# mburger-stsci/nexoclom

Hardware: AMD Instinct MI355X
Metric: particle*steps/s (higher is better)
Workload: dtype f64

## Files before the change

### nexoclom_amd/csrc/nxc_api.hip

```cpp
#include <hip/hip_runtime.h>
#include <dlfcn.h>
#include <rccl/rccl.h>

#include <algorithm>
#include <atomic>
#include <cmath>
#include <cstddef>
#include <cstdio>
#include <cstdlib>
#include <cstring>
#include <ctime>
#include <limits>
#include <mutex>
#include <new>
#include <string>
#include <utility>
#include <vector>

#include "../../include/nexoclom_hip.h"
#include "nxc_camera_check.hpp"
#include "nxc_shell_check.hpp"
#include "nxc_cube_check.hpp"
#include "nxc_los_profile_check.hpp"
#include "nxc_desc_check.hpp"
// ... 2571 lines not shown
        K.n_node_az = rows(ST_NODE_AZ);
    }
    HIPCHK(hipMemsetAsync(h->d_ctr, 0, sizeof(DevCounters), h->stream));
    if ((rc = begin_timed(h))) return rc;
    const auto kernel = plan.law == NXC_LAW_NODES ? k_sample<NXC_LAW_NODES>
                        : (plan.law == NXC_LAW_THERMAL ? k_sample<NXC_LAW_THERMAL> : k_sample<NXC_LAW_PLAIN>);
    hipLaunchKernelGGL(kernel, dim3(flat_grid(h, n, NXC_BLOCK)), dim3(NXC_BLOCK), 0, h->stream, K, n,
                       h->d_packets, h->d_ctr);
    HIPCHK(hipGetLastError());
    if ((rc = end_timed(h))) return rc;
    DevCounters c;
    HIPCHK(hipMemcpyAsync(&c, h->d_ctr, sizeof c, hipMemcpyDeviceToHost, h->stream));
    HIPCHK(stream_sync(h));
    if (c.unfinished) {
        h->n_packets = 0;
        h->have_order = false;
        return fail(NXC_ERR_ARG, "nxc_packets_sample: " + std::to_string(c.unfinished) +
                                 " packets found no launch point in the density map (is it "
                                 "almost everywhere zero?)");
    }
    h->n_packets = total;
    h->var_n = -1;
    h->rows_total = -1;
    if (offset == 0) h->first_id = d->first_index;
    h->have_order = false;
    if (soa_out)
        HIPCHK(hipMemcpy2DAsync(soa_out, (size_t)n * 8, h->d_packets + offset, (size_t)total * 8,
                                (size_t)n * 8, 8, hipMemcpyDeviceToHost, h->stream));
    if (offset + n < total) {
        HIPCHK(stream_sync(h));
        return NXC_OK;
    }
    if ((rc = order_on_device(h, plan.k2max, nullptr, 0))) return rc;
    HIPCHK(stream_sync(h));
    return NXC_OK;
    });
}

int nxc_integrate_const_async(nxc_handle *h, double step, int64_t n_iter, double outeredge,
                              uint32_t flags)
{
    return guarded([&]() -> int {
    int rc = need_forces(h);
    if (rc) return rc;
    if (h->n_packets < 1) return fail(NXC_ERR_STATE, "no resident packets (nxc_packets_upload)");
    if (!(step > 0) || n_iter < 0) return fail(NXC_ERR_ARG, "step must be > 0, n_iter >= 0");
    const bool image = (flags & NXC_RUN_IMAGE) != 0;
    if (image && !h->have_image) return fail(NXC_ERR_STATE, "NXC_RUN_IMAGE without nxc_set_image");
    if ((rc = speed_order_for_const(h))) return rc;
    return launch_const(h, step, n_iter, outeredge, image, nullptr, nullptr);
    });
}

int nxc_integrate_const_streamed(nxc_handle *h, int64_t n, const double *soa0, int32_t pieces,
                                 double step, int64_t n_iter, double outeredge, uint32_t flags)
{
    return guarded([&]() -> int {
    int rc = need_forces(h);
    if (rc) return rc;
    if (n < 1 || !soa0 || pieces < 1 || pieces > 32) return fail(NXC_ERR_ARG, "bad arguments (1..32 pieces)");
    if (!(step > 0) || n_iter < 0) return fail(NXC_ERR_ARG, "step must be > 0, n_iter >= 0");
    const bool image = (flags & NXC_RUN_IMAGE) != 0;
    if (image && !h->have_image) return fail(NXC_ERR_STATE, "NXC_RUN_IMAGE without nxc_set_image");
    if (n >= (int64_t)0xffffffffll) return fail(NXC_ERR_ARG, "too many packets for one resident set");
    if (h->have_bodies || h->have_bounce)
        return fail(NXC_ERR_STATE, "the streamed pass covers the plain force models; with moons or "
                                   "surface re-emission upload first (nxc_packets_upload)");
    if ((int64_t)pieces > n) pieces = (int32_t)n;
    const size_t per_piece = NXC_ORDER_BINS + 8;
    if ((rc = h->d_packets.ensure((size_t)8 * n * 8))) return rc;
    if ((rc = h->d_queue.ensure((size_t)8 * n * 8))) return rc;
    if ((rc = h->d_order.ensure((size_t)n * sizeof(unsigned)))) return rc;
    if ((rc = h->d_piece_hist.ensure((32 * per_piece + 8) * sizeof(unsigned long long)))) return rc;
    for (int e = 0; e <= 32; e++)
        if (!h->ev_piece[e]) HIPCHK(hipEventCreateWithFlags(&h->ev_piece[e], hipEventDisableTiming));
    unsigned long long *d_avail = h->d_piece_hist + 32 * per_piece;
    h->n_packets = n;
    h->var_n = -1;
    h->first_id = 0;
    h->rows_total = -1;
    h->have_order = false;

    if ((rc = upload_step(h, step))) return rc;
    HIPCHK(hipMemsetAsync(h->d_ctr, 0, sizeof(DevCounters), h->stream));
    HIPCHK(hipMemsetAsync(d_avail, 0, sizeof(unsigned long long), h->stream));
    HIPCHK(hipEventRecord(h->ev_piece[32], h->stream));
    HIPCHK(hipStreamWaitEvent(h->stream2, h->ev_piece[32], 0));
    HIPCHK(hipStreamWaitEvent(h->copy_stream, h->ev_piece[32], 0));
    FusedJob job;
    job.soa = h->d_queue; job.order = h->d_order; job.avail = d_avail;
    if ((rc = launch_fused(h, image, 0, n_iter, outeredge, job))) return rc;
    auto give_up = [&](int code) {
        hipLaunchKernelGGL(k_publish, dim3(1), dim3(64), 0, h->stream2, d_avail, ~0ull);
        (void)hipStreamSynchronize(h->stream2);
        (void)stream_sync(h);
        h->n_packets = 0;
        return code;
    };
    std::vector<int64_t> bound((size_t)pieces + 1, n);
    bound[0] = 0;
    if (pieces > 1) {
        int64_t first = std::max<int64_t>(n / (4 * (int64_t)pieces), (int64_t)h->n_cu * BLOCK_PERSIST * 2);
        first = std::min(first, n / pieces);
        for (int p = 1; p < pieces; p++) bound[(size_t)p] = first + (n - first) * (p - 1) / (pieces - 1);
    }
    const bool withhold = std::getenv("NXC_TEST_WITHHOLD_LAST_PIECE") != nullptr;
    for (int p = 0; p < pieces; p++) {
        const int64_t p0 = bound[(size_t)p], len = bound[(size_t)p + 1] - p0;
        if (len <= 0) continue;
        if (withhold && p == pieces - 1 && pieces > 1) break;
        hipError_t e = hipSuccess;
        for (int c = 0; c < 8 && e == hipSuccess; c++)
            e = hipMemcpyAsync(h->d_packets + c * n + p0, soa0 + c * n + p0, (size_t)len * 8,
                               hipMemcpyHostToDevice, h->copy_stream);
        if (e == hipSuccess) e = hipEventRecord(h->ev_piece[p], h->copy_stream);
        if (e == hipSuccess) e = hipStreamWaitEvent(h->stream2, h->ev_piece[p], 0);
        unsigned long long *hist = h->d_piece_hist + (size_t)p * per_piece, *d_max = hist + NXC_ORDER_BINS;
        if (e == hipSuccess) e = hipMemsetAsync(d_max, 0, sizeof(unsigned long long), h->stream2);
        if (e != hipSuccess)
            return give_up(fail_hip("streamed upload", e));
        hipLaunchKernelGGL(k_speed_max<false>, dim3(flat_grid(h, len, NXC_BLOCK)), dim3(NXC_BLOCK), 0,
                           h->stream2, (const double *)(h->d_packets + p0), n, len, d_max);
        if ((rc = order_async(h, h->stream2, h->d_packets + p0, n, len, nullptr, 0.0, d_max, hist,
                              h->d_order + p0, h->d_queue + 8 * p0, true, (unsigned)p0)))
            return give_up(rc);
        hipLaunchKernelGGL(k_publish, dim3(1), dim3(64), 0, h->stream2, d_avail,
                           (unsigned long long)(p0 + len));
        if (hipGetLastError() != hipSuccess) return give_up(fail(NXC_ERR_HIP, "streamed upload: launch failed"));
    }
    h->have_order = true;
    h->order_key = 0;
    h->streamed_pending = true;
    HIPCHK(hipEventRecord(h->ev_piece[32], h->stream2));
    HIPCHK(hipStreamWaitEvent(h->stream, h->ev_piece[32], 0));
    return NXC_OK;
    });
}

int nxc_integrate_const(nxc_handle *h, double step, int64_t n_iter, double outeredge,
                        uint32_t flags, double *traj_out, int64_t nrec, double *final_out,
                        int64_t *steps_out)
{
    return guarded([&]() -> int {
    int rc = need_forces(h);
    if (rc) return rc;
    const int64_t n = h->n_packets;
    if (n < 1) return fail(NXC_ERR_STATE, "no resident packets (nxc_packets_upload)");
    if (!(step > 0) || n_iter < 0) return fail(NXC_ERR_ARG, "step must be > 0, n_iter >= 0");
    const bool image = (flags & NXC_RUN_IMAGE) != 0;
    if (image && !h->have_image) return fail(NXC_ERR_STATE, "NXC_RUN_IMAGE without nxc_set_image");
    if (traj_out && nrec < n_iter + 1) return fail(NXC_ERR_ARG, "nrec must be >= n_iter + 1");
    if ((rc = speed_order_for_const(h))) return rc;

    const size_t col = (size_t)n * sizeof(double);
    double *d_final = nullptr;
    long long *d_steps = nullptr;
    if (!traj_out) {
        if (final_out) {
            if ((rc = scratch_for(h, 8 * col)))
                return rc;
            d_final = h->d_scratch;
        }
        if (steps_out) {
            if ((rc = h->d_steps.ensure((size_t)n * sizeof(long long))))
                return rc;
            d_steps = h->d_steps;
        }
        if ((rc = launch_const(h, step, n_iter, outeredge, image, d_final, d_steps))) return rc;
    } else {
        const size_t tbytes = (size_t)8 * (size_t)nrec * col;
        size_t free_b = 0, total_b = 0;
        HIPCHK(hipMemGetInfo(&free_b, &total_b));
        if (tbytes > free_b && pool_bytes(h)) {
            pool_flush(h);
            HIPCHK(hipMemGetInfo(&free_b, &total_b));
        }
        if (tbytes > free_b)
            return fail(NXC_ERR_ARG, "trajectory buffer does not fit in device memory; run fewer "
// ... 1509 lines not shown
```

### nexoclom_amd/csrc/nxc_device.hpp

```cpp
#pragma once
#include <hip/hip_runtime.h>
#include <stdint.h>
#include "nxc_math.hpp"
#include "nxc_fused_variant.hpp"

struct LutDesc {
    int rec, fs, cell;
    int top;
    int last;
    int pad_;
    double xbase;
    double inv_w;
};
typedef LutDesc LutView;

extern __shared__ __align__(32) unsigned char nxc_lds[];

#define NXC_LDS_AS __attribute__((address_space(3)))
#define NXC_GLOBAL_AS __attribute__((address_space(1)))
typedef double nxc_v2d __attribute__((ext_vector_type(2)));

NXC_DEV double lds_f64(int byte_off)
{
    return *(const NXC_LDS_AS double *)(unsigned)byte_off;
// ... 253 lines not shown
            const double bd = Tableau::B5[i] - Tableau::B4[i];
            e[0] = nxc_tab_fma(bd, kv[i][0], e[0]);
            e[1] = nxc_tab_fma(bd, kv[i][1], e[1]);
            e[2] = nxc_tab_fma(bd, kv[i][2], e[2]);
            e[3] = nxc_tab_fma(bd, ka[i][0], e[3]);
            e[4] = nxc_tab_fma(bd, ka[i][1], e[4]);
            e[5] = nxc_tab_fma(bd, ka[i][2], e[5]);
            e[6] = nxc_tab_fma(bd, kl[i], e[6]);
        }
        d[0] = 0.0;
#pragma unroll
        for (int c = 0; c < 7; c++) d[c + 1] = __builtin_fabs(h * e[c]);
    }
    s[0] = (-h) + s[0];
    s[1] = px; s[2] = py; s[3] = pz; s[4] = vx; s[5] = vy; s[6] = vz;
    s[7] = nxc_exp(lf);
}

struct ImageK {
    double M[9];
    double vrplanet, apix_cm2;
    int quantity, n_lines, downcast_f32, dbg;
    int nx, nz;
    int x_is_x, pad_;
    double x_lo, x_inv_step, z_lo, z_inv_step;
    int64_t xedges_off, zedges_off;
    LutDesc line[4];
};

struct BounceK {
    double GM, unit_km, accom, stickcoef, A0, A1, A2, t0, t1;
    int temp_dependent, nx, ny, pad_;
    unsigned long long seed;
    const double *tx, *ty, *coef;
    const double *mlon, *mlat, *mcoef;
    int mlon_n, mlat_n;
};

struct LoopK {
    const double *soa0;
    const unsigned *order;
    double *final_out;
    long long *steps_out;
    unsigned long long *head;
    long long n;
    const long long *offsets;
    const unsigned long long *avail;
    long long q_rec, q_col;
};
struct WeightK {
    double rs_1e6, rs_apix;
};

constexpr int NXC_LOG_BINS = 91;
struct LdsHeader {
    ImageK G;
    StepW W;
    BounceK B;
    BodyK Bd;
    LoopK L;
    WeightK Wt;
    alignas(32) double logtab[NXC_LOG_BINS][4];
};
constexpr int NXC_HEADER_BYTES = (int)((sizeof(LdsHeader) + 31) & ~size_t(31));

NXC_DEV const LdsHeader &lds_header()
{
    return *reinterpret_cast<const LdsHeader *>(nxc_lds);
}

NXC_DEV double nxc_log(double x)
{
    constexpr double LN2_HI = 6.93147180369123816490e-01, LN2_LO = 1.90821492927058770002e-10;
    constexpr double OFF = 0.70703125;
    int k = 0;
    if (__builtin_expect(!(x >= 2.2250738585072014e-308 && x <= 1.7976931348623157e308), 0)) {
        if (x != x) return x;
        if (x == 0.0) return -__builtin_huge_val();
        if (x < 0.0) return __builtin_nan("");
        if (x == __builtin_huge_val()) return x;
        x *= 18014398509481984.0; k = -54;
    }
    const int hx = __double2hiint(x);
    const int tmp = hx - 0x3FE6A000;
    k += tmp >> 20;
    const double m = __hiloint2double(hx - (int)((unsigned)tmp & 0xFFF00000u), __double2loint(x));
    const int i = (int)((m - OFF) * 128.0);
    const int row = (int)offsetof(LdsHeader, logtab) + 32 * i;
    const double2 t01 = lds_f64x2(row);
    const double lclo = lds_f64(row + 16);
    const double r = __builtin_fma(m, t01.x, -1.0);
    const double kd = (double)k;
    const double w = __builtin_fma(kd, LN2_HI, t01.y);
    const double hi = w + r;
    const double lo = ((w - hi) + r) + __builtin_fma(kd, LN2_LO, lclo);
    double p = -0x1.999999999999ap-4;
    p = __builtin_fma(p, r, nxc_sconst(0x1.c71c71c71c71cp-4));
    p = __builtin_fma(p, r, nxc_sconst(-0x1.0p-3));
    p = __builtin_fma(p, r, nxc_sconst(0x1.2492492492492p-3));
    p = __builtin_fma(p, r, nxc_sconst(-0x1.5555555555555p-3));
    p = __builtin_fma(p, r, nxc_sconst(0x1.999999999999ap-3));
    p = __builtin_fma(p, r, nxc_sconst(-0x1.0p-2));
    p = __builtin_fma(p, r, nxc_sconst(0x1.5555555555555p-2));
    return __builtin_fma(r * r, __builtin_fma(r, p, -0.5), lo) + hi;
}
NXC_DEV LdsHeader &lds_header_rw()
{
    return *reinterpret_cast<LdsHeader *>(nxc_lds);
}

NXC_DEV void philox4x32_10(unsigned c0, unsigned c1, unsigned c2, unsigned c3, unsigned k0,
                           unsigned k1, unsigned (&out)[4])
{
#pragma unroll
// ... 670 lines not shown
```

### nexoclom_amd/csrc/nxc_kernels.hpp

```cpp
#pragma once
#include "nxc_device.hpp"
#include "nxc_fused_variant.hpp"
#include "nxc_source_limits.hpp"
#include "nxc_tile_plan.hpp"

struct DevCounters {
    unsigned long long particle_steps, samples, samples_binned, nonfinite, bad_step, neg_frac,
        unfinished, queue_head;
    unsigned long long wave_trips;
#ifdef NXC_STAMPS
    unsigned long long stamp[8];
#endif
};

#ifdef NXC_STAMPS
NXC_DEV unsigned long long nxc_stamp()
{
    unsigned long long t;
    __builtin_amdgcn_sched_barrier(0);
    asm volatile("s_memtime %0\n\ts_waitcnt lgkmcnt(0)" : "=s"(t) : : "memory");
    __builtin_amdgcn_sched_barrier(0);
    return t;
}
#define NXC_STAMP(k) do { const unsigned long long t_ = nxc_stamp(); seg[k] += t_ - t_prev; t_prev = t_; } while (0)
#else
#define NXC_STAMP(k) do { } while (0)
#endif

constexpr int NXC_BLOCK = 256;

NXC_DEV void stage_tables(const unsigned char *__restrict__ blob, int64_t bytes)
{
    if ((unsigned)(size_t)(NXC_LDS_AS unsigned char *)nxc_lds != 0u) __builtin_trap();
    const unsigned long long *src = reinterpret_cast<const unsigned long long *>(blob);
    unsigned long long *dst = reinterpret_cast<unsigned long long *>(nxc_lds);
    const int64_t words = bytes >> 3;
    for (int64_t w = threadIdx.x; w < words; w += blockDim.x) dst[w] = src[w];
    __syncthreads();
    if (threadIdx.x == 0) {
        LdsHeader &H = lds_header_rw();
        H.Wt.rs_1e6 = nxc_recip_seed(1e6);
        H.Wt.rs_apix = nxc_mid_range(H.G.apix_cm2) ? nxc_recip_seed(H.G.apix_cm2)
                                                   : __builtin_nan("");
    }
    __syncthreads();
}

NXC_DEV void stage_tables_and_args(const unsigned char *__restrict__ blob, int64_t bytes,
                                   const double *soa0, const unsigned *order, double *final_out,
                                   long long *steps_out, unsigned long long *head, long long n,
                                   const long long *offsets = nullptr,
                                   const unsigned long long *avail = nullptr)
{
    stage_tables(blob, bytes);
    if (threadIdx.x == 0) {
// ... 134 lines not shown
__global__ void __launch_bounds__(NXC_TR_ROWS)
k_rows_transpose(const void *__restrict__ rec_, long long total, T *__restrict__ cols,
                 I *__restrict__ index)
{
    static_assert(sizeof(T) == sizeof(I), "a record is ten equal-sized slots");
    typedef T pair_t __attribute__((ext_vector_type(2)));
    __shared__ pair_t tile[NXC_TR_ROWS * 5];
    const T *rec = static_cast<const T *>(rec_);
    for (long long base = (long long)blockIdx.x * NXC_TR_ROWS; base < total;
         base += (long long)gridDim.x * NXC_TR_ROWS) {
        const int nrow = (int)((total - base) < NXC_TR_ROWS ? (total - base) : NXC_TR_ROWS);
        const pair_t *src = reinterpret_cast<const pair_t *>(rec + base * 10);
        for (int w = threadIdx.x; w < nrow * 5; w += NXC_TR_ROWS) tile[w] = src[w];
        __syncthreads();
        if ((int)threadIdx.x < nrow) {
            const T *r = reinterpret_cast<const T *>(tile) + threadIdx.x * 10;
            const long long row = base + threadIdx.x;
#pragma unroll
            for (int c = 0; c < 9; c++) cols[c * total + row] = r[c];
            I id;
            __builtin_memcpy(&id, &r[9], sizeof id);
            index[row] = id;
        }
        __syncthreads();
    }
}

constexpr int NXC_DENSIFY_RECORDS = 32;
__global__ void __launch_bounds__(NXC_BLOCK)
k_rows_densify(const double *__restrict__ rec, const long long *__restrict__ offsets,
               const double *__restrict__ final_soa, const long long *__restrict__ steps,
               int64_t n, int64_t nrec, double *__restrict__ traj)
{
    const int64_t i = (int64_t)blockIdx.x * blockDim.x + threadIdx.x;
    if (i >= n) return;
    const long long off = offsets[i], len = offsets[i + 1] - off, last = steps[i];
    const int64_t k0 = (int64_t)blockIdx.y * NXC_DENSIFY_RECORDS;
    const int64_t k1 = k0 + NXC_DENSIFY_RECORDS < nrec ? k0 + NXC_DENSIFY_RECORDS : nrec;
    for (int64_t k = k0; k < k1; k++) {
        double v[8] = {0, 0, 0, 0, 0, 0, 0, 0};
        if (k < len) {
            const nxc_v2d *r = reinterpret_cast<const nxc_v2d *>(rec + (off + k) * NXC_REC_DOUBLES);
#pragma unroll
            for (int c = 0; c < 4; c++) { const nxc_v2d t = r[c]; v[2 * c] = t.x; v[2 * c + 1] = t.y; }
        } else if (k == last) {
#pragma unroll
            for (int c = 0; c < 8; c++) v[c] = final_soa[c * n + i];
        }
#pragma unroll
        for (int c = 0; c < 8; c++) traj[((int64_t)c * nrec + k) * n + i] = v[c];
    }
}

NXC_DEV bool wait_published(const unsigned long long *avail, unsigned long long need)
{
    unsigned long long t0 = 0;
    bool timing = false;
    for (;;) {
        const unsigned long long v =
            __hip_atomic_load(avail, __ATOMIC_ACQUIRE, __HIP_MEMORY_SCOPE_AGENT);
        if (v == ~0ull) return false;
        if (v >= need) return true;
        const unsigned long long now = __builtin_amdgcn_s_memrealtime();
        if (!timing) { t0 = now; timing = true; }
        else if (now - t0 > 300000000ull) return false;
        __builtin_amdgcn_s_sleep(32);
    }
}

__global__ void k_publish(unsigned long long *avail, unsigned long long value)
{
    if (threadIdx.x == 0 && blockIdx.x == 0)
        __hip_atomic_store(avail, value, __ATOMIC_RELEASE, __HIP_MEMORY_SCOPE_AGENT);
}

struct WaveQueue {
    long long pending = 0;
    int c_pos = 0, c_cnt = 0;
    bool drained = false, stalled = false;

    static NXC_DEV long long claim(unsigned long long *head)
    {
        return (long long)__hip_atomic_fetch_add((NXC_GLOBAL_AS unsigned long long *)head,
                                                 (unsigned long long)NXC_CHUNK, __ATOMIC_RELAXED,
                                                 __HIP_MEMORY_SCOPE_AGENT);
    }

    NXC_DEV void start()
    {
        if ((threadIdx.x & 63) == 0) pending = claim(lds_header().L.head);
    }

    template <bool ROWS = false, bool STREAMED = false>
    NXC_DEV long long refill(bool need, int stage_off, double (&s)[8], long long *row0 = nullptr,
                             long long *nrow = nullptr)
    {
        const unsigned long long mask = __ballot(need);
        long long mine = -1;
        if (mask == 0 || drained) return mine;
        const int want = __popcll(mask);
        const int lane = threadIdx.x & 63;
        const int rank = __popcll(mask & ((1ull << lane) - 1ull));
        NXC_LDS_AS double *stage = (NXC_LDS_AS double *)(unsigned)stage_off;
        int served = 0;
        while (served < want) {
            if (c_pos >= c_cnt) {
                const LoopK &L = lds_header().L;
                const long long n = L.n;
                const double *__restrict__ soa0 = L.soa0;
                const unsigned *__restrict__ ids = L.order;
                const long long b = wave_bcast0(pending);
                if (b >= n) { drained = true; break; }
                c_cnt = (b + NXC_CHUNK <= n) ? NXC_CHUNK : (int)(n - b);
                c_pos = 0;
                if (STREAMED) {
                    if (!wait_published(L.avail, (unsigned long long)(b + c_cnt))) {
                        drained = true; stalled = true; c_cnt = 0;
                        break;
                    }
                }
                __builtin_amdgcn_fence(__ATOMIC_RELEASE, "wavefront");
                if (lane < c_cnt) {
                    const long long q_col = L.q_col;
                    const NXC_GLOBAL_AS double *g = (const NXC_GLOBAL_AS double *)soa0 + (b + lane) * L.q_rec;
                    const NXC_GLOBAL_AS unsigned *gid = (const NXC_GLOBAL_AS unsigned *)ids;
                    double col[8];
#pragma unroll
                    for (int c = 0; c < 8; c++) col[c] = g[c * q_col];
                    const long long pid = gid ? (long long)gid[b + lane] : b + lane;
                    long long o0 = 0, o1 = 0;
                    if (ROWS) {
                        const NXC_GLOBAL_AS long long *offs = (const NXC_GLOBAL_AS long long *)L.offsets;
                        o0 = offs[pid]; o1 = offs[pid + 1];
                    }
#pragma unroll
                    for (int c = 0; c < 8; c++) stage[c * NXC_CHUNK + lane] = col[c];
                    stage[8 * NXC_CHUNK + lane] = __longlong_as_double(pid);
                    if (ROWS) {
                        stage[9 * NXC_CHUNK + lane] = __longlong_as_double(o0);
                        stage[10 * NXC_CHUNK + lane] = __longlong_as_double(o1 - o0);
                    }
                }
                if (lane == 0) pending = claim(L.head);
                __builtin_amdgcn_fence(__ATOMIC_ACQUIRE, "wavefront");
                __builtin_amdgcn_wave_barrier();
            }
            const int room = c_cnt - c_pos;
            const int take = room < (want - served) ? room : want - served;
            if (need && rank >= served && rank < served + take) {
                const int slot = c_pos + (rank - served);
                mine = __double_as_longlong(stage[8 * NXC_CHUNK + slot]);
#pragma unroll
                for (int c = 0; c < 8; c++) s[c] = stage[c * NXC_CHUNK + slot];
                if (ROWS) {
                    *row0 = __double_as_longlong(stage[9 * NXC_CHUNK + slot]);
                    *nrow = __double_as_longlong(stage[10 * NXC_CHUNK + slot]);
                }
            }
            c_pos += take;
            served += take;
        }
        return mine;
    }
};

template <int IMAGE>
NXC_DEV bool image_pop(ImageQueue &queue, int imgq_off, const ImageRegs &IR, int &p, double &rv,
                       double &fw, unsigned long long &nonfinite)
{
    if (IMAGE == 2) {
        double x = 0, y = 0, z = 0, vy = 0, frac = 0;
        const bool ok = queue.pop_sample(imgq_off, x, y, z, vy, frac);
        if (ok) p = image_locate_core(lds_header().G, IR, x, y, z, vy, frac, rv, fw, nonfinite);
        return ok && p >= 0;
    }
    return queue.pop(imgq_off, p, rv, fw);
}

template <int IMAGE, bool BOUNCE, bool FULL, bool NBODY = false, int ROWS = 0, bool STREAMED = false>
__global__ void __launch_bounds__(NXC_BLOCK_PERSIST)
k_const_fused(ForceK F, const unsigned char *__restrict__ blob,
              int64_t stage_bytes, int64_t n, const double *__restrict__ soa0,
              const unsigned *__restrict__ order, int64_t first_id, int64_t n_iter,
              double edge2, double *__restrict__ final_out,
              long long *__restrict__ steps_out, double *__restrict__ acc2,
              DevCounters *__restrict__ ctr, const double *__restrict__ moon_pos = nullptr,
              const long long *__restrict__ offsets = nullptr, void *__restrict__ rec = nullptr,
              const unsigned long long *__restrict__ avail = nullptr)
{
    static_assert(!(IMAGE && ROWS), "the rows pass has no image");
    static_assert(!(STREAMED && (ROWS || BOUNCE || NBODY)), "the streamed pass is the plain one");
    stage_tables_and_args(blob, stage_bytes, soa0, order, final_out, steps_out, &ctr->queue_head, n,
                          offsets, STREAMED ? avail : nullptr);
    const LutView T = lut_view(F.tab);
    ImageRegs IR{};
    if (IMAGE) IR = image_regs(lds_header().G);
    ImageQueue queue;
    unsigned my_steps = 0, my_samples = 0, my_binned = 0;
    unsigned long long my_nonfinite = 0;
    WaveQueue q;
    q.start();
    const bool want_out = __builtin_amdgcn_readfirstlane(
        (final_out != nullptr || steps_out != nullptr) ? 1 : 0) != 0;
    const int wave_off = (int)((stage_bytes + 31) & ~31ll) +
                         (threadIdx.x >> 6) * (ROWS ? NXC_WAVE_LDS_BYTES_ROWS : NXC_WAVE_LDS_BYTES);
    const int stage_off = wave_off, imgq_off = wave_off + NXC_WAVE_STAGE_BYTES;
    bool has = false, fresh = false;
    long long id = -1, row0 = 0, nrow = 0;
    double lossfrac = 0.0;
    unsigned my_overrun = 0, my_trips = 0;
    int k = 0, nbounce = 0;
    const int n_it = n_iter > 0x7fffffffll ? 0x7fffffff : (int)n_iter;
    double s[8], d[8];
#ifdef NXC_STAMPS
    unsigned long long seg[8] = {0, 0, 0, 0, 0, 0, 0, 0}, t_prev = nxc_stamp();
#endif
    for (;;) {
#ifdef NXC_REFILL_MIN
        const unsigned long long free_ = __ballot(!has);
        const bool serve = __popcll(free_) >= NXC_REFILL_MIN || free_ == ~0ull;
        const long long got = serve ? q.refill<ROWS != 0, STREAMED>(!has, stage_off, s, &row0, &nrow) : -1;
#else
        const long long got = q.refill<ROWS != 0, STREAMED>(!has, stage_off, s, &row0, &nrow);
#endif
        if (got >= 0) { id = got; k = 0; has = true; fresh = true; nbounce = 0; lossfrac = 0.0; }
        if (__ballot(has) == 0) break;
        my_trips++;
        NXC_STAMP(0);
        int p = -1;
        double rv = 0.0, fw = 0.0;
        bool inframe = false;
        float qx = 0.f, qy = 0.f, qz = 0.f;
        if (has) {
            const double before = s[7];
            if (!fresh) {
                if (NBODY) {
                    const BodyK *Bd = &lds_header().Bd;
                    const double *mp = moon_pos + (long long)k * (2 * Bd->n_moons);
                    rk5_step<false, true, FULL, true>(F, T, s, 0.0, lds_header().W, d, Bd, mp);
                    apply_fate<false, true>(s, edge2, 0ull, nbounce, my_nonfinite, Bd, mp);
                } else {
                    rk5_step<false, true, FULL>(F, T, s, 0.0, lds_header().W, d);
                    apply_fate<BOUNCE>(s, edge2, (unsigned long long)(first_id + id), nbounce, my_nonfinite);
                }
#ifdef NXC_PROBE_VMOV
                {
// ... 1624 lines not shown
            my_unfinished += !accepted;
        }
        const double clat = cos(lat);
        const double x0 = (K.is_planet ? 1.0 : -1.0) * K.exobase * sin(lon) * clat;
        const double y0 = -K.exobase * cos(lon) * clat;
        const double z0 = K.exobase * sin(lat);
        double v;
        if (K.speed_type == 0) {
            v = uspd * 2 * K.vwidth + K.vprob - K.vwidth;
        } else if (K.speed_type == 1) {
            double g0, g1;
            philox_pair(gi, 3, NXC_STREAM_SOURCE, K.seed, g0, g1);
            const double zn = sqrt(-2.0 * log(1.0 - g0)) * cos(TWO_PI * g1);
            v = K.vwidth == 0.0 ? K.vprob : zn * K.vwidth + K.vprob;
        } else if (THERMAL) {
            double tsurf = K.t0;
            if (lon <= 1.5707963267948966 || lon >= 4.71238898038469)
                tsurf = K.t0 + K.t1 * nxc_sqrt(nxc_sqrt(__builtin_fabs(cos(lon) * cos(lat))));
            const double s = bispev3(K.spl, tsurf, uspd);
            v = s > 0.0 ? s : 0.0;
        } else if (NODES && K.speed_type == 4) {
            v = interp_node(K.node_speed_cdf, K.node_speed_v, K.n_node_speed, node, uspd);
        } else {
            v = interp_global(K.speed_cdf, K.speed_v, K.n_speed, uspd);
        }
        v = v / K.unit_km;
        double alt, az;
        if (NODES && K.angular_type == 2) {
            alt = interp_node(K.node_alt_cdf, K.node_alt, K.n_node_alt, node, ualt);
            az = interp_node(K.node_az_cdf, K.node_az, K.n_node_az, node, uaz);
        } else if (K.angular_type == 0) {
            alt = 1.5707963267948966; az = 0.0;
        } else {
            alt = asin(ualt * (K.sinalt1 - K.sinalt0) + K.sinalt0);
            az = K.az0 + (K.az1 - K.az0) * uaz;
        }
        const double v_rad = sin(alt), v_t0 = cos(alt) * cos(az), v_t1 = cos(alt) * sin(az);
        const double rn = sqrt((x0 * x0 + y0 * y0) + z0 * z0);
        const double en = sqrt(y0 * y0 + x0 * x0);
        const double n0 = -z0 * x0, n1 = -z0 * y0, n2 = x0 * x0 + y0 * y0;
        const double nn = sqrt((n0 * n0 + n1 * n1) + n2 * n2);
        const double dx = (v_t0 * (n0 / nn) + v_t1 * (y0 / en)) + v_rad * (x0 / rn);
        const double dy = (v_t0 * (n1 / nn) + v_t1 * (-x0 / en)) + v_rad * (y0 / rn);
        const double dz = (v_t0 * (n2 / nn) + v_t1 * 0.0) + v_rad * (z0 / rn);
        double *__restrict__ dst = soa + K.offset + i;
        dst[0] = time;
        dst[1 * K.stride] = x0; dst[2 * K.stride] = y0; dst[3 * K.stride] = z0;
        dst[4 * K.stride] = dx * v; dst[5 * K.stride] = dy * v; dst[6 * K.stride] = dz * v;
        dst[7 * K.stride] = 1.0;
    }
    flush_counter(&ctr->unfinished, my_unfinished);
}

constexpr int NXC_ORDER_BINS = 4096;

NXC_DEV int steps_bin(const long long *__restrict__ steps, int64_t i, double scale)
{
    const double f = (double)steps[i] * scale;
    int b = f < (double)NXC_ORDER_BINS ? (int)f : NXC_ORDER_BINS - 1;
    return NXC_ORDER_BINS - 1 - (b < 0 ? 0 : b);
}

NXC_DEV int speed_bin(const double *__restrict__ soa, int64_t stride, int64_t i, double scale)
{
    const double vx = soa[4 * stride + i], vy = soa[5 * stride + i], vz = soa[6 * stride + i];
    const double f = (vx * vx + vy * vy + vz * vz) * scale;
    int b = (f >= 0.0 && f < (double)NXC_ORDER_BINS) ? (int)f : (f >= (double)NXC_ORDER_BINS ? NXC_ORDER_BINS - 1 : 0);
    return NXC_ORDER_BINS - 1 - b;
}

NXC_DEV double flight_key(const double *__restrict__ soa, int64_t stride, int64_t i)
{
    const double vx = soa[4 * stride + i], vy = soa[5 * stride + i], vz = soa[6 * stride + i];
    return soa[i] / __builtin_sqrt(vx * vx + vy * vy + vz * vz);
}
NXC_DEV int flight_bin(const double *__restrict__ soa, int64_t stride, int64_t i, double scale)
{
    const double f = flight_key(soa, stride, i) * scale;
    int b = (f >= 0.0 && f < (double)NXC_ORDER_BINS) ? (int)f : (f >= (double)NXC_ORDER_BINS ? NXC_ORDER_BINS - 1 : 0);
    return NXC_ORDER_BINS - 1 - b;
}
template <int KEY>
NXC_DEV int order_bin(const double *__restrict__ soa, const long long *__restrict__ steps, int64_t stride,
                      int64_t i, double scale)
{
    return KEY == 1 ? steps_bin(steps, i, scale) : KEY == 2 ? flight_bin(soa, stride, i, scale)
                                                              : speed_bin(soa, stride, i, scale);
}

NXC_DEV double order_scale(double scale, const unsigned long long *__restrict__ max_bits)
{
    if (!max_bits) return scale;
    const double m = __longlong_as_double((long long)*max_bits);
    return m > 0.0 ? (double)(NXC_ORDER_BINS - 1) / m : 0.0;
}

template <bool FLIGHT = false>
__global__ void __launch_bounds__(NXC_BLOCK)
k_speed_max(const double *__restrict__ soa, int64_t stride, int64_t n, unsigned long long *__restrict__ out)
{
    double m = 0.0;
    for (int64_t i = (int64_t)blockIdx.x * blockDim.x + threadIdx.x; i < n;
         i += (int64_t)gridDim.x * blockDim.x) {
        const double vx = soa[4 * stride + i], vy = soa[5 * stride + i], vz = soa[6 * stride + i];
        const double f = FLIGHT ? flight_key(soa, stride, i) : vx * vx + vy * vy + vz * vz;
        if (f <= 1.7976931348623157e308 && f > m) m = f;
    }
#pragma unroll
    for (int off = 32; off > 0; off >>= 1) {
        const double o = __shfl_down(m, off, 64);
        m = o > m ? o : m;
    }
    if ((threadIdx.x & 63) == 0 && m > 0.0)
        atomicMax(out, (unsigned long long)__double_as_longlong(m));
}

template <int KEY, bool LDS>
__global__ void __launch_bounds__(NXC_BLOCK)
k_order_hist(const double *__restrict__ soa, const long long *__restrict__ steps, int64_t stride,
             int64_t n, double scale_, const unsigned long long *__restrict__ max_bits,
             unsigned long long *__restrict__ hist)
{
    const double scale = order_scale(scale_, max_bits);
    if (LDS) {
        __shared__ unsigned lh[NXC_ORDER_BINS];
        for (int b = threadIdx.x; b < NXC_ORDER_BINS; b += blockDim.x) lh[b] = 0;
        __syncthreads();
        for (int64_t i = (int64_t)blockIdx.x * blockDim.x + threadIdx.x; i < n;
             i += (int64_t)gridDim.x * blockDim.x)
            atomicAdd(&lh[order_bin<KEY>(soa, steps, stride, i, scale)], 1u);
        __syncthreads();
        for (int b = threadIdx.x; b < NXC_ORDER_BINS; b += blockDim.x)
            if (lh[b]) atomicAdd(&hist[b], (unsigned long long)lh[b]);
    } else {
        for (int64_t i = (int64_t)blockIdx.x * blockDim.x + threadIdx.x; i < n;
             i += (int64_t)gridDim.x * blockDim.x)
            atomicAdd(&hist[order_bin<KEY>(soa, steps, stride, i, scale)], 1ull);
    }
}

__global__ void __launch_bounds__(64)
k_order_scan(unsigned long long *__restrict__ hist)
{
    constexpr int PER = NXC_ORDER_BINS / 64;
    const int lane = threadIdx.x;
    unsigned long long sum = 0;
    for (int j = 0; j < PER; j++) sum += hist[lane * PER + j];
    unsigned long long incl = sum;
#pragma unroll
    for (int off = 1; off < 64; off <<= 1) {
        const unsigned long long o = __shfl_up(incl, off, 64);
        if (lane >= off) incl += o;
    }
    unsigned long long acc = incl - sum;
    for (int j = 0; j < PER; j++) {
        const unsigned long long v = hist[lane * PER + j];
        hist[lane * PER + j] = acc;
        acc += v;
    }
}

template <int KEY>
__global__ void __launch_bounds__(NXC_BLOCK)
k_order_scatter(const double *__restrict__ soa, const long long *__restrict__ steps, int64_t stride,
                int64_t n, double scale_, const unsigned long long *__restrict__ max_bits,
                unsigned long long *__restrict__ cursor, unsigned *__restrict__ order, unsigned base,
                double *__restrict__ queue)
{
    const double scale = order_scale(scale_, max_bits);
    for (int64_t i = (int64_t)blockIdx.x * blockDim.x + threadIdx.x; i < n;
         i += (int64_t)gridDim.x * blockDim.x) {
        double v[8];
#pragma unroll
        for (int c = 0; c < 8; c++) v[c] = soa[c * stride + i];
        const unsigned long long pos =
            atomicAdd(&cursor[order_bin<KEY>(soa, steps, stride, i, scale)], 1ull);
        order[pos] = base + (unsigned)i;
        nxc_v2d *rec = reinterpret_cast<nxc_v2d *>(queue + 8 * pos);
#pragma unroll
        for (int c = 0; c < 4; c++) { nxc_v2d t; t.x = v[2 * c]; t.y = v[2 * c + 1]; rec[c] = t; }
    }
}

__global__ void k_sum_counters(const DevCounters *__restrict__ pieces, int n, DevCounters *__restrict__ out)
{
    if (threadIdx.x == 0 && blockIdx.x == 0) {
        DevCounters t{};
        for (int p = 0; p < n; p++) {
            t.particle_steps += pieces[p].particle_steps; t.samples += pieces[p].samples;
            t.samples_binned += pieces[p].samples_binned; t.nonfinite += pieces[p].nonfinite;
            t.bad_step += pieces[p].bad_step; t.neg_frac += pieces[p].neg_frac;
            t.unfinished += pieces[p].unfinished; t.wave_trips += pieces[p].wave_trips;
        }
        *out = t;
    }
}

struct DensityK {
    double o[3];
    double inv_h;
    double r_cell;
    double dr2;
    int n[3];
    int reserved;
};

NXC_DEV bool density_cells(const DensityK &K, const double p[3], int lo[3], int hi[3])
{
#pragma unroll
    for (int a = 0; a < 3; a++) {
        const double t = (p[a] - K.o[a]) * K.inv_h;
// ... 593 lines not shown
```

Measured before the change: 33.20 billion.

## Streamlined per-piece binning and LDS-shared publish polling in streamed integration

Replaces the per-piece speed-max, histogram, scan and scatter sequence with two kernels. A histogram kernel bins by speed-squared float bits, which removes the max pass, and its last-arriving block scans only the occupied bin range. The consumer waits on published pieces through an LDS-cached value that one elected wave polls with exponential backoff, cutting global atomic polling traffic from every wave. It also zeroes all piece histograms up front and makes the first-piece size configurable. The risks are many more bins (64K) per piece and subtler memory-ordering behaviour.

```diff
diff --git a/nexoclom_amd/csrc/nxc_api.hip b/nexoclom_amd/csrc/nxc_api.hip
--- a/nexoclom_amd/csrc/nxc_api.hip
+++ b/nexoclom_amd/csrc/nxc_api.hip
@@ -2647,6 +2647,9 @@
     });
 }
 
+#ifndef NXC_STREAM_FIRST_PER_LANE
+#define NXC_STREAM_FIRST_PER_LANE 2
+#endif
 int nxc_integrate_const_streamed(nxc_handle *h, int64_t n, const double *soa0, int32_t pieces,
                                  double step, int64_t n_iter, double outeredge, uint32_t flags)
 {
@@ -2662,14 +2665,14 @@
         return fail(NXC_ERR_STATE, "the streamed pass covers the plain force models; with moons or "
                                    "surface re-emission upload first (nxc_packets_upload)");
     if ((int64_t)pieces > n) pieces = (int32_t)n;
-    const size_t per_piece = NXC_ORDER_BINS + 8;
+    const size_t per_piece = NXC_PIECE_WORDS;
     if ((rc = h->d_packets.ensure((size_t)8 * n * 8))) return rc;
     if ((rc = h->d_queue.ensure((size_t)8 * n * 8))) return rc;
     if ((rc = h->d_order.ensure((size_t)n * sizeof(unsigned)))) return rc;
-    if ((rc = h->d_piece_hist.ensure((32 * per_piece + 8) * sizeof(unsigned long long)))) return rc;
+    if ((rc = h->d_piece_hist.ensure((8 + 32 * per_piece) * sizeof(unsigned long long)))) return rc;
     for (int e = 0; e <= 32; e++)
         if (!h->ev_piece[e]) HIPCHK(hipEventCreateWithFlags(&h->ev_piece[e], hipEventDisableTiming));
-    unsigned long long *d_avail = h->d_piece_hist + 32 * per_piece;
+    unsigned long long *d_avail = h->d_piece_hist;
     h->n_packets = n;
     h->var_n = -1;
     h->first_id = 0;
@@ -2678,7 +2681,8 @@
 
     if ((rc = upload_step(h, step))) return rc;
     HIPCHK(hipMemsetAsync(h->d_ctr, 0, sizeof(DevCounters), h->stream));
-    HIPCHK(hipMemsetAsync(d_avail, 0, sizeof(unsigned long long), h->stream));
+    HIPCHK(hipMemsetAsync(h->d_piece_hist, 0, (8 + (size_t)pieces * per_piece) * sizeof(unsigned long long),
+                          h->stream));
     HIPCHK(hipEventRecord(h->ev_piece[32], h->stream));
     HIPCHK(hipStreamWaitEvent(h->stream2, h->ev_piece[32], 0));
     HIPCHK(hipStreamWaitEvent(h->copy_stream, h->ev_piece[32], 0));
@@ -2695,7 +2699,8 @@
     std::vector<int64_t> bound((size_t)pieces + 1, n);
     bound[0] = 0;
     if (pieces > 1) {
-        int64_t first = std::max<int64_t>(n / (4 * (int64_t)pieces), (int64_t)h->n_cu * BLOCK_PERSIST * 2);
+        int64_t first = std::max<int64_t>(n / (4 * (int64_t)pieces),
+                                          (int64_t)h->n_cu * BLOCK_PERSIST * NXC_STREAM_FIRST_PER_LANE);
         first = std::min(first, n / pieces);
         for (int p = 1; p < pieces; p++) bound[(size_t)p] = first + (n - first) * (p - 1) / (pieces - 1);
     }
@@ -2710,15 +2715,15 @@
                                hipMemcpyHostToDevice, h->copy_stream);
         if (e == hipSuccess) e = hipEventRecord(h->ev_piece[p], h->copy_stream);
         if (e == hipSuccess) e = hipStreamWaitEvent(h->stream2, h->ev_piece[p], 0);
-        unsigned long long *hist = h->d_piece_hist + (size_t)p * per_piece, *d_max = hist + NXC_ORDER_BINS;
-        if (e == hipSuccess) e = hipMemsetAsync(d_max, 0, sizeof(unsigned long long), h->stream2);
         if (e != hipSuccess)
             return give_up(fail_hip("streamed upload", e));
-        hipLaunchKernelGGL(k_speed_max<false>, dim3(flat_grid(h, len, NXC_BLOCK)), dim3(NXC_BLOCK), 0,
-                           h->stream2, (const double *)(h->d_packets + p0), n, len, d_max);
-        if ((rc = order_async(h, h->stream2, h->d_packets + p0, n, len, nullptr, 0.0, d_max, hist,
-                              h->d_order + p0, h->d_queue + 8 * p0, true, (unsigned)p0)))
-            return give_up(rc);
+        unsigned long long *hist = h->d_piece_hist + 8 + (size_t)p * per_piece;
+        const int grid = flat_grid(h, len, NXC_BLOCK);
+        hipLaunchKernelGGL(k_piece_hist, dim3(grid), dim3(NXC_BLOCK), 0, h->stream2,
+                           (const double *)(h->d_packets + p0), n, len, hist);
+        hipLaunchKernelGGL(k_piece_scatter, dim3(grid), dim3(NXC_BLOCK), 0, h->stream2,
+                           (const double *)(h->d_packets + p0), n, len, hist, h->d_order + p0,
+                           (unsigned)p0, h->d_queue + 8 * p0);
         hipLaunchKernelGGL(k_publish, dim3(1), dim3(64), 0, h->stream2, d_avail,
                            (unsigned long long)(p0 + len));
         if (hipGetLastError() != hipSuccess) return give_up(fail(NXC_ERR_HIP, "streamed upload: launch failed"));
diff --git a/nexoclom_amd/csrc/nxc_device.hpp b/nexoclom_amd/csrc/nxc_device.hpp
--- a/nexoclom_amd/csrc/nxc_device.hpp
+++ b/nexoclom_amd/csrc/nxc_device.hpp
@@ -329,6 +329,13 @@
     double rs_1e6, rs_apix;
 };
 
+struct StreamK {
+    unsigned long long seen;
+    unsigned poller;
+    unsigned reserved;
+};
+static_assert(sizeof(StreamK) == 16, "StreamK takes the place of the padding in front of logtab");
+
 constexpr int NXC_LOG_BINS = 91;
 struct LdsHeader {
     ImageK G;
@@ -337,6 +344,7 @@
     BodyK Bd;
     LoopK L;
     WeightK Wt;
+    StreamK S;
     alignas(32) double logtab[NXC_LOG_BINS][4];
 };
 constexpr int NXC_HEADER_BYTES = (int)((sizeof(LdsHeader) + 31) & ~size_t(31));
diff --git a/nexoclom_amd/csrc/nxc_kernels.hpp b/nexoclom_amd/csrc/nxc_kernels.hpp
--- a/nexoclom_amd/csrc/nxc_kernels.hpp
+++ b/nexoclom_amd/csrc/nxc_kernels.hpp
@@ -1,6 +1,7 @@
 #pragma once
 #include "nxc_device.hpp"
 #include "nxc_fused_variant.hpp"
+#include "nxc_order_key.hpp"
 #include "nxc_source_limits.hpp"
 #include "nxc_tile_plan.hpp"
 
@@ -241,20 +242,66 @@
     }
 }
 
-NXC_DEV bool wait_published(const unsigned long long *avail, unsigned long long need)
-{
-    unsigned long long t0 = 0;
-    bool timing = false;
+#ifndef NXC_POLL_NAP_CAP
+#define NXC_POLL_NAP_CAP 8
+#endif
+NXC_DEV bool published_in_lds(unsigned long long need)
+{
+    const unsigned long long v = (unsigned long long)wave_bcast0((long long)__hip_atomic_load(
+        &lds_header_rw().S.seen, __ATOMIC_ACQUIRE, __HIP_MEMORY_SCOPE_WORKGROUP));
+    return v != ~0ull && v >= need;
+}
+
+template <typename T> NXC_DEV T nxc_in_vgpr(T x)
+{
+    asm volatile("" : "+v"(x));
+    return x;
+}
+
+#ifdef NXC_WAIT_NOINLINE
+__attribute__((noinline))
+#endif
+NXC_DEV bool wait_published(unsigned long long need_)
+{
+    StreamK &S = lds_header_rw().S;
+    const bool lane0 = (threadIdx.x & 63) == 0;
+    const unsigned long long need = nxc_in_vgpr(need_);
+    unsigned long long t0 = nxc_in_vgpr(0ull);
+    int poller = nxc_in_vgpr(0), ok = nxc_in_vgpr(0), nap = nxc_in_vgpr(1);
     for (;;) {
-        const unsigned long long v =
-            __hip_atomic_load(avail, __ATOMIC_ACQUIRE, __HIP_MEMORY_SCOPE_AGENT);
-        if (v == ~0ull) return false;
-        if (v >= need) return true;
-        const unsigned long long now = __builtin_amdgcn_s_memrealtime();
-        if (!timing) { t0 = now; timing = true; }
-        else if (now - t0 > 300000000ull) return false;
-        __builtin_amdgcn_s_sleep(32);
-    }
+        unsigned long long v = 0;
+        if (!poller) {
+            v = __hip_atomic_load(&S.seen, __ATOMIC_ACQUIRE, __HIP_MEMORY_SCOPE_WORKGROUP);
+            if (v == ~0ull) break;
+            if (v >= need) { ok = 1; break; }
+            int got = 0;
+            if (lane0) {
+                unsigned expected = 0u;
+                got = __hip_atomic_compare_exchange_strong(&S.poller, &expected, 1u, __ATOMIC_ACQUIRE,
+                                                           __ATOMIC_RELAXED, __HIP_MEMORY_SCOPE_WORKGROUP);
+            }
+            poller = nxc_in_vgpr(__builtin_amdgcn_readfirstlane(got));
+        }
+        if (poller) {
+            if (lane0) {
+                v = __hip_atomic_load((const NXC_GLOBAL_AS unsigned long long *)lds_header().L.avail,
+                                      __ATOMIC_ACQUIRE, __HIP_MEMORY_SCOPE_AGENT);
+                __hip_atomic_store(&S.seen, v, __ATOMIC_RELEASE, __HIP_MEMORY_SCOPE_WORKGROUP);
+            }
+            v = nxc_in_vgpr((unsigned long long)wave_bcast0((long long)v));
+            if (v == ~0ull) break;
+            if (v >= need) { ok = 1; break; }
+        }
+        const unsigned long long now = nxc_in_vgpr((unsigned long long)__builtin_amdgcn_s_memrealtime());
+        if (t0 == 0ull) t0 = now;
+        else if (now - t0 > 300000000ull) break;
+        const int naps = __builtin_amdgcn_readfirstlane(nap);
+        for (int i = 0; i < naps; i++) __builtin_amdgcn_s_sleep(32);
+        if (poller && nap < NXC_POLL_NAP_CAP) nap <<= 1;
+    }
+    if (poller && lane0)
+        __hip_atomic_store(&S.poller, 0u, __ATOMIC_RELEASE, __HIP_MEMORY_SCOPE_WORKGROUP);
+    return __builtin_amdgcn_readfirstlane(ok) != 0;
 }
 
 __global__ void k_publish(unsigned long long *avail, unsigned long long value)
@@ -303,7 +350,8 @@
                 c_cnt = (b + NXC_CHUNK <= n) ? NXC_CHUNK : (int)(n - b);
                 c_pos = 0;
                 if (STREAMED) {
-                    if (!wait_published(L.avail, (unsigned long long)(b + c_cnt))) {
+                    const unsigned long long need = (unsigned long long)(b + c_cnt);
+                    if (!published_in_lds(need) && !wait_published(need)) {
                         drained = true; stalled = true; c_cnt = 0;
                         break;
                     }
@@ -381,6 +429,13 @@
     static_assert(!(STREAMED && (ROWS || BOUNCE || NBODY)), "the streamed pass is the plain one");
     stage_tables_and_args(blob, stage_bytes, soa0, order, final_out, steps_out, &ctr->queue_head, n,
                           offsets, STREAMED ? avail : nullptr);
+    if (STREAMED) {
+        if (threadIdx.x == 0) {
+            StreamK &S = lds_header_rw().S;
+            S.seen = 0ull; S.poller = 0u;
+        }
+        __syncthreads();
+    }
     const LutView T = lut_view(F.tab);
     ImageRegs IR{};
     if (IMAGE) IR = image_regs(lds_header().G);
@@ -2111,7 +2166,6 @@
     flush_counter(&ctr->unfinished, my_unfinished);
 }
 
-constexpr int NXC_ORDER_BINS = 4096;
 
 NXC_DEV int steps_bin(const long long *__restrict__ steps, int64_t i, double scale)
 {
@@ -2198,11 +2252,10 @@
     }
 }
 
-__global__ void __launch_bounds__(64)
-k_order_scan(unsigned long long *__restrict__ hist)
+NXC_DEV void order_scan_wave(unsigned long long *__restrict__ hist)
 {
     constexpr int PER = NXC_ORDER_BINS / 64;
-    const int lane = threadIdx.x;
+    const int lane = threadIdx.x & 63;
     unsigned long long sum = 0;
     for (int j = 0; j < PER; j++) sum += hist[lane * PER + j];
     unsigned long long incl = sum;
@@ -2216,6 +2269,103 @@
         const unsigned long long v = hist[lane * PER + j];
         hist[lane * PER + j] = acc;
         acc += v;
+    }
+}
+__global__ void __launch_bounds__(64)
+k_order_scan(unsigned long long *__restrict__ hist)
+{
+    order_scan_wave(hist);
+}
+
+constexpr int NXC_PIECE_TICKET = NXC_PIECE_BINS, NXC_PIECE_HI = NXC_PIECE_BINS + 1,
+              NXC_PIECE_LO = NXC_PIECE_BINS + 2, NXC_PIECE_WORDS = NXC_PIECE_BINS + 8;
+
+NXC_DEV int piece_bin(double vx, double vy, double vz)
+{
+    return nxc_speed_queue_bin((uint64_t)__double_as_longlong(vx * vx + vy * vy + vz * vz));
+}
+
+NXC_DEV int wave_max(int v)
+{
+#pragma unroll
+    for (int off = 32; off > 0; off >>= 1) {
+        const int o = __shfl_down(v, off, 64);
+        v = o > v ? o : v;
+    }
+    return v;
+}
+
+__global__ void __launch_bounds__(NXC_BLOCK)
+k_piece_hist(const double *__restrict__ soa, int64_t stride, int64_t n, unsigned long long *hist)
+{
+    int hi = -1, lo = -1;
+    for (int64_t i = (int64_t)blockIdx.x * blockDim.x + threadIdx.x; i < n;
+         i += (int64_t)gridDim.x * blockDim.x) {
+        const int b = piece_bin(soa[4 * stride + i], soa[5 * stride + i], soa[6 * stride + i]);
+        __hip_atomic_fetch_add(&hist[b], 1ull, __ATOMIC_RELAXED, __HIP_MEMORY_SCOPE_AGENT);
+        hi = b > hi ? b : hi;
+        lo = NXC_PIECE_BINS - 1 - b > lo ? NXC_PIECE_BINS - 1 - b : lo;
+    }
+    hi = wave_max(hi); lo = wave_max(lo);
+    if ((threadIdx.x & 63) == 0 && hi >= 0) {
+        __hip_atomic_fetch_max(&hist[NXC_PIECE_HI], (unsigned long long)hi, __ATOMIC_RELAXED,
+                               __HIP_MEMORY_SCOPE_AGENT);
+        __hip_atomic_fetch_max(&hist[NXC_PIECE_LO], (unsigned long long)lo, __ATOMIC_RELAXED,
+                               __HIP_MEMORY_SCOPE_AGENT);
+    }
+    __builtin_amdgcn_fence(__ATOMIC_RELEASE, "agent");
+    __syncthreads();
+    if (threadIdx.x >= 64) return;
+    unsigned long long ticket = 0;
+    if (threadIdx.x == 0)
+        ticket = __hip_atomic_fetch_add(&hist[NXC_PIECE_TICKET], 1ull, __ATOMIC_ACQ_REL,
+                                        __HIP_MEMORY_SCOPE_AGENT);
+    ticket = (unsigned long long)wave_bcast0((long long)ticket);
+    if (ticket != (unsigned long long)gridDim.x - 1ull) return;
+    __builtin_amdgcn_fence(__ATOMIC_ACQUIRE, "agent");
+    const int lane = threadIdx.x;
+    int first = NXC_PIECE_BINS - 1 - (int)hist[NXC_PIECE_LO], last = (int)hist[NXC_PIECE_HI];
+    first = first < 0 ? 0 : first;
+    last = last > NXC_PIECE_BINS - 1 ? NXC_PIECE_BINS - 1 : last;
+    constexpr int TILES = 8;
+    unsigned long long carry = 0;
+    for (int base = first & ~63; base <= last; base += 64 * TILES) {
+        unsigned long long v[TILES], incl[TILES];
+#pragma unroll
+        for (int u = 0; u < TILES; u++)
+            v[u] = base + 64 * u <= last ? hist[base + 64 * u + lane] : 0ull;
+#pragma unroll
+        for (int u = 0; u < TILES; u++) {
+            incl[u] = v[u];
+#pragma unroll
+            for (int off = 1; off < 64; off <<= 1) {
+                const unsigned long long o = __shfl_up(incl[u], off, 64);
+                if (lane >= off) incl[u] += o;
+            }
+        }
+#pragma unroll
+        for (int u = 0; u < TILES; u++) {
+            if (base + 64 * u <= last) hist[base + 64 * u + lane] = carry + incl[u] - v[u];
+            carry += __shfl(incl[u], 63, 64);
+        }
+    }
+}
+
+__global__ void __launch_bounds__(NXC_BLOCK)
+k_piece_scatter(const double *__restrict__ soa, int64_t stride, int64_t n,
+                unsigned long long *__restrict__ cursor, unsigned *__restrict__ order, unsigned base,
+                double *__restrict__ queue)
+{
+    for (int64_t i = (int64_t)blockIdx.x * blockDim.x + threadIdx.x; i < n;
+         i += (int64_t)gridDim.x * blockDim.x) {
+        double v[8];
+#pragma unroll
+        for (int c = 0; c < 8; c++) v[c] = soa[c * stride + i];
+        const unsigned long long pos = atomicAdd(&cursor[piece_bin(v[4], v[5], v[6])], 1ull);
+        order[pos] = base + (unsigned)i;
+        nxc_v2d *rec = reinterpret_cast<nxc_v2d *>(queue + 8 * pos);
+#pragma unroll
+        for (int c = 0; c < 4; c++) { nxc_v2d t; t.x = v[2 * c]; t.y = v[2 * c + 1]; rec[c] = t; }
     }
 }
 
diff --git a/nexoclom_amd/csrc/nxc_order_key.hpp b/nexoclom_amd/csrc/nxc_order_key.hpp
--- /dev/null
+++ b/nexoclom_amd/csrc/nxc_order_key.hpp
@@ -0,0 +1,21 @@
+#pragma once
+#include <cstdint>
+
+constexpr int NXC_ORDER_BINS = 4096;
+constexpr int NXC_KEY_MANT = 10;
+constexpr int NXC_KEY_LOW_EXP = -56;
+constexpr int NXC_PIECE_BINS = 64 << NXC_KEY_MANT;
+
+constexpr int nxc_speed_key(uint64_t v2_bits)
+{
+    constexpr uint64_t INF = 0x7ff0000000000000ull;
+    if ((v2_bits >> 63) != 0 || v2_bits > INF) return 0;
+    const int64_t k = (int64_t)(v2_bits >> (52 - NXC_KEY_MANT)) -
+                      (int64_t)(1023 + NXC_KEY_LOW_EXP) * (1 << NXC_KEY_MANT);
+    return k < 0 ? 0 : (k > NXC_PIECE_BINS - 1 ? NXC_PIECE_BINS - 1 : (int)k);
+}
+
+constexpr int nxc_speed_queue_bin(uint64_t v2_bits)
+{
+    return NXC_PIECE_BINS - 1 - nxc_speed_key(v2_bits);
+}
```

After: 33.47 billion (median of 2 runs). Within noise of the previous version (+0.8%).
